# RupertLuo/Valley

Hardware: AMD Instinct MI355X
Metric: frames/sec ViT-L/14 encode + prefill tokens/sec (13B) (higher is better)
Workload: dtype bf16

## Files before the change

valley_amd/csrc/gemm_skinny.hip:

```cpp
#include <cstdlib>
#include "common.hpp"
#include "../../include/valley_hip.h"

namespace {

constexpr int SK_UNROLL = 4;

template <int EPI, int NWV>
__global__ void __launch_bounds__(NWV * 64) gemm_skinny_kernel(const uint16_t* __restrict__ A, const uint16_t* __restrict__ W,
                                                               const float* __restrict__ bias, uint16_t* __restrict__ C, int M, int N,
                                                               int K, int lda, int ldw, int ldc) {
    __shared__ f32x4 red[NWV][4][64];
    const int tid = threadIdx.x, lane = tid & 63, wave = tid >> 6;
    const int l15 = lane & 15, g = lane >> 4;
    const int n0 = blockIdx.x * 32, m0 = blockIdx.y * 32;
    const int kq = K / NWV, kbeg = wave * kq;
    const uint16_t* a0 = A + (size_t)min(m0 + l15, M - 1) * lda + kbeg + g * 8;
    const uint16_t* a1 = A + (size_t)min(m0 + 16 + l15, M - 1) * lda + kbeg + g * 8;
    const uint16_t* w0 = W + (size_t)(n0 + l15) * ldw + kbeg + g * 8;
    const uint16_t* w1 = W + (size_t)(n0 + 16 + l15) * ldw + kbeg + g * 8;
    f32x4 acc[2][2];
#pragma unroll
    for (int i = 0; i < 2; ++i)
#pragma unroll
        for (int j = 0; j < 2; ++j) acc[i][j] = f32x4{0.f, 0.f, 0.f, 0.f};
    const int groups = (kq % (32 * SK_UNROLL) == 0) ? kq / (32 * SK_UNROLL) : 0;
    if (groups > 0) {
        bf16x8 fa0[SK_UNROLL], fa1[SK_UNROLL], fw0[SK_UNROLL], fw1[SK_UNROLL];
        auto load_group = [&](bf16x8 (&xa0)[SK_UNROLL], bf16x8 (&xa1)[SK_UNROLL], bf16x8 (&xw0)[SK_UNROLL], bf16x8 (&xw1)[SK_UNROLL],
                              int k) {
#pragma unroll
            for (int u = 0; u < SK_UNROLL; ++u) {
                xw0[u] = *(const bf16x8*)(w0 + k + 32 * u);
                xw1[u] = *(const bf16x8*)(w1 + k + 32 * u);
                xa0[u] = *(const bf16x8*)(a0 + k + 32 * u);
                xa1[u] = *(const bf16x8*)(a1 + k + 32 * u);
            }
        };
        auto mfma_group = [&](const bf16x8 (&xa0)[SK_UNROLL], const bf16x8 (&xa1)[SK_UNROLL], const bf16x8 (&xw0)[SK_UNROLL],
                              const bf16x8 (&xw1)[SK_UNROLL]) {
#pragma unroll
            for (int u = 0; u < SK_UNROLL; ++u) {
                acc[0][0] = mfma16(xw0[u], xa0[u], acc[0][0]);
                acc[0][1] = mfma16(xw1[u], xa0[u], acc[0][1]);
                acc[1][0] = mfma16(xw0[u], xa1[u], acc[1][0]);
                acc[1][1] = mfma16(xw1[u], xa1[u], acc[1][1]);
            }
        };
        load_group(fa0, fa1, fw0, fw1, 0);
        if constexpr (NWV == 4) {
            bf16x8 ga0[SK_UNROLL], ga1[SK_UNROLL], gw0[SK_UNROLL], gw1[SK_UNROLL];
#pragma unroll 1
            for (int it = 0; it < groups; it += 2) {
                if (it + 1 < groups) load_group(ga0, ga1, gw0, gw1, (it + 1) * 32 * SK_UNROLL);
                mfma_group(fa0, fa1, fw0, fw1);
                if (it + 1 >= groups) break;
                if (it + 2 < groups) load_group(fa0, fa1, fw0, fw1, (it + 2) * 32 * SK_UNROLL);
                mfma_group(ga0, ga1, gw0, gw1);
            }
        } else {
#pragma unroll 1
            for (int it = 0; it < groups; ++it) {
                mfma_group(fa0, fa1, fw0, fw1);
                if (it + 1 < groups) load_group(fa0, fa1, fw0, fw1, (it + 1) * 32 * SK_UNROLL);
            }
        }
    } else
    for (int k = 0; k < kq; k += 32 * SK_UNROLL) {
        bf16x8 fa0[SK_UNROLL], fa1[SK_UNROLL], fw0[SK_UNROLL], fw1[SK_UNROLL];
#pragma unroll
        for (int u = 0; u < SK_UNROLL; ++u) {
            const int kk = min(k + 32 * u, kq - 32);
            fa0[u] = *(const bf16x8*)(a0 + kk);
            fa1[u] = *(const bf16x8*)(a1 + kk);
            fw0[u] = *(const bf16x8*)(w0 + kk);
            fw1[u] = *(const bf16x8*)(w1 + kk);
        }
#pragma unroll
        for (int u = 0; u < SK_UNROLL; ++u) {
            if (k + 32 * u < kq) {
                acc[0][0] = mfma16(fw0[u], fa0[u], acc[0][0]);
                acc[0][1] = mfma16(fw1[u], fa0[u], acc[0][1]);
                acc[1][0] = mfma16(fw0[u], fa1[u], acc[1][0]);
                acc[1][1] = mfma16(fw1[u], fa1[u], acc[1][1]);
            }
        }
    }
#pragma unroll
    for (int i = 0; i < 2; ++i)
#pragma unroll
        for (int j = 0; j < 2; ++j) red[wave][2 * i + j][lane] = acc[i][j];
    __syncthreads();
    if (wave >= 4) return;
    f32x4 v = red[0][wave][lane];
#pragma unroll
    for (int w = 1; w < NWV; ++w) v += red[w][wave][lane];
    const int m = m0 + (wave >> 1) * 16 + l15, n = n0 + (wave & 1) * 16 + 4 * g;
    if (m >= M) return;
    if (bias) v += *(const f32x4*)(bias + n);
    if constexpr (EPI == VLY_EPI_QUICK_GELU) {
#pragma unroll
        for (int r = 0; r < 4; ++r) v[r] = x_sigmoid(v[r], 1.702f);
    }
    if constexpr (EPI == VLY_EPI_RELU) {
#pragma unroll
        for (int r = 0; r < 4; ++r) v[r] = fmaxf(v[r], 0.f);
    }
    u32x2 pk;
    pk[0] = pack_h2(v[0], v[1]);
    pk[1] = pack_h2(v[2], v[3]);
    *(u32x2*)(C + (size_t)m * ldc + n) = pk;
}

}

extern "C" int vly_gemm_skinny_bf16(const void* A, const void* W, const float* bias, void* C, int M, int N, int K, int lda, int ldw,
                                    int ldc, int epilogue, void* stream) {
    if (M <= 0 || M > 256 || N <= 0 || N % 32 || K < 128 || K % 128 || (K >= 2048 && K % 512) || lda % 8 || ldw % 8 || ldc % 4 || ((uintptr_t)A & 15) ||
        ((uintptr_t)W & 15) || ((uintptr_t)C & 7) || (bias && ((uintptr_t)bias & 15))) {
        vly_set_error("vly_gemm_skinny_bf16: unsupported shape/alignment M=%d N=%d K=%d lda=%d ldw=%d ldc=%d", M, N, K, lda, ldw, ldc);
        return -22;
    }
    static const bool narrow_only = getenv("VLY_SKINNY_WAVES") && atoi(getenv("VLY_SKINNY_WAVES")) == 4;
    const bool wide = K >= 2048 && !narrow_only;
    dim3 grid(N / 32, (M + 31) / 32), block(wide ? 1024 : 256);
    hipStream_t st = (hipStream_t)stream;
#define VLY_SKINNY(E)                                                                                                      \
    do {                                                                                                                   \
        if (wide)                                                                                                          \
            hipLaunchKernelGGL((gemm_skinny_kernel<E, 16>), grid, block, 0, st, (const uint16_t*)A, (const uint16_t*)W, bias,  \
                               (uint16_t*)C, M, N, K, lda, ldw, ldc);                                                      \
        else                                                                                                               \
            hipLaunchKernelGGL((gemm_skinny_kernel<E, 4>), grid, block, 0, st, (const uint16_t*)A, (const uint16_t*)W, bias,   \
                               (uint16_t*)C, M, N, K, lda, ldw, ldc);                                                      \
    } while (0)
    switch (epilogue) {
        case VLY_EPI_NONE: VLY_SKINNY(VLY_EPI_NONE); break;
        case VLY_EPI_QUICK_GELU: VLY_SKINNY(VLY_EPI_QUICK_GELU); break;
        case VLY_EPI_RELU: VLY_SKINNY(VLY_EPI_RELU); break;
        default: vly_set_error("vly_gemm_skinny_bf16: unsupported epilogue %d", epilogue); return -22;
    }
#undef VLY_SKINNY
    return vly_check_launch("vly_gemm_skinny_bf16");
}
```

Before: 1717.

## Stage skinny GEMM operands through LDS with direct buffer-to-LDS loads and slot ring

Adds a new skinny GEMM kernel that streams W and A tiles into per-wave LDS rings using buffer_load ... lds with counted vmcnt waits. Operands are then read back through XOR-swizzled LDS addresses. A 16-row M tile variant is used when M is small or the grid is underfilled. This path becomes the default and is meant to replace strided per-lane global vector loads with wide coalesced row loads and deeper prefetch. The trade-off is hand-written inline asm with manual wait counting and a tighter M lower bound (M<=8 now rejected).

```diff
diff --git a/valley_amd/csrc/gemm_skinny.hip b/valley_amd/csrc/gemm_skinny.hip
--- a/valley_amd/csrc/gemm_skinny.hip
+++ b/valley_amd/csrc/gemm_skinny.hip
@@ -112,11 +112,121 @@
     *(u32x2*)(C + (size_t)m * ldc + n) = pk;
 }
 
+template <int EPI, int NWV, int BM, int NSLOT>
+__global__ void __launch_bounds__(NWV * 64) gemm_skinny_lines_kernel(const uint16_t* __restrict__ A, const uint16_t* __restrict__ W,
+                                                                     const float* __restrict__ bias, uint16_t* __restrict__ C, int M, int N,
+                                                                     int K, int lda, int ldw, int ldc) {
+    constexpr int FM = BM / 16;
+    constexpr int PW = 4, PA = BM / 8, PIECES = PW + PA;
+    constexpr int SLOT = PIECES * 1024;
+    static_assert((NSLOT - 1) * PIECES < 64 && NSLOT >= 1 && NSLOT <= 4, "vmcnt is six bits; the counted waits below cover four slots");
+    static_assert(2 * FM * 1024 <= SLOT, "the reduction buffer of a wave lives in its own ring");
+    __shared__ __attribute__((aligned(16))) char ring[NWV][NSLOT][SLOT];
+    const int tid = threadIdx.x, lane = tid & 63, wave = __builtin_amdgcn_readfirstlane(tid >> 6);
+    const int l15 = lane & 15, g = lane >> 4;
+    const int n0 = blockIdx.x * 32, m0 = blockIdx.y * BM;
+    const int kq = K / NWV, kbeg = wave * kq;
+    const int nst = (kq + 63) >> 6;
+    const int r8 = lane >> 3, ch = (lane & 7) ^ r8;
+    const __amdgpu_buffer_rsrc_t rsW = vly_rsrc(W + (size_t)n0 * ldw), rsA = vly_rsrc(A + (size_t)m0 * lda);
+    uint32_t voW[PW], voA[PA];
+#pragma unroll
+    for (int q = 0; q < PW; ++q) voW[q] = ((uint32_t)(q * 8 + r8) * (uint32_t)ldw + (uint32_t)ch * 8u) * 2u;
+#pragma unroll
+    for (int q = 0; q < PA; ++q) voA[q] = ((uint32_t)(min(m0 + q * 8 + r8, M - 1) - m0) * (uint32_t)lda + (uint32_t)ch * 8u) * 2u;
+    const uint32_t half_back = (uint32_t)(ch & 4) * 16u;
+    char* my = &ring[wave][0][0];
+    const uint32_t my_lds = __builtin_amdgcn_readfirstlane((uint32_t)(uintptr_t)(__attribute__((address_space(3))) char*)my);
+    auto dma = [&](uint32_t voff, __amdgpu_buffer_rsrc_t rs, uint32_t soff, uint32_t dst) {
+        asm volatile("s_mov_b32 m0, %3\n\ts_nop 0\n\tbuffer_load_dwordx4 %0, %1, %2 offen lds" ::"v"(voff), "s"(rs), "s"(soff), "s"(dst)
+                     : "memory");
+    };
+    auto issue = [&](int step) {
+        const uint32_t d = my_lds + (uint32_t)(step % NSLOT) * SLOT, soff = (uint32_t)(kbeg + step * 64) * 2u;
+        const uint32_t back = (step * 64 + 32 >= kq) ? half_back : 0u;
+#pragma unroll
+        for (int q = 0; q < PW; ++q) dma(voW[q] - back, rsW, soff, d + q * 1024);
+#pragma unroll
+        for (int q = 0; q < PA; ++q) dma(voA[q] - back, rsA, soff, d + (PW + q) * 1024);
+    };
+    const int rd[2] = {l15 * 128 + (((0 + g) ^ (l15 & 7)) << 4), l15 * 128 + (((4 + g) ^ (l15 & 7)) << 4)};
+    f32x4 acc[FM][2];
+#pragma unroll
+    for (int i = 0; i < FM; ++i)
+#pragma unroll
+        for (int j = 0; j < 2; ++j) acc[i][j] = f32x4{0.f, 0.f, 0.f, 0.f};
+#pragma unroll
+    for (int s = 0; s < NSLOT; ++s)
+        if (s < nst) issue(s);
+#pragma unroll 1
+    for (int i = 0; i < nst; ++i) {
+        const int younger = min(nst - 1 - i, NSLOT - 1);
+        if (NSLOT > 3 && younger == 3) asm volatile("s_waitcnt vmcnt(%0)" ::"i"(NSLOT > 3 ? 3 * PIECES : 0) : "memory");
+        else if (NSLOT > 2 && younger == 2) asm volatile("s_waitcnt vmcnt(%0)" ::"i"(NSLOT > 2 ? 2 * PIECES : 0) : "memory");
+        else if (NSLOT > 1 && younger == 1) asm volatile("s_waitcnt vmcnt(%0)" ::"i"(PIECES) : "memory");
+        else asm volatile("s_waitcnt vmcnt(0)" ::: "memory");
+        const char* s = my + (i % NSLOT) * SLOT;
+        bf16x8 fw[2][2], fa[FM][2];
+#pragma unroll
+        for (int u = 0; u < 2; ++u) {
+#pragma unroll
+            for (int j = 0; j < 2; ++j) fw[j][u] = *(const bf16x8*)(s + j * 2048 + rd[u]);
+#pragma unroll
+            for (int f = 0; f < FM; ++f) fa[f][u] = *(const bf16x8*)(s + PW * 1024 + f * 2048 + rd[u]);
+        }
+        asm volatile("s_waitcnt lgkmcnt(0)" ::: "memory");
+        if (i + NSLOT < nst) issue(i + NSLOT);
+#pragma unroll
+        for (int u = 0; u < 2; ++u) {
+            if (i * 64 + 32 * u < kq) {
+#pragma unroll
+                for (int f = 0; f < FM; ++f)
+#pragma unroll
+                    for (int j = 0; j < 2; ++j) acc[f][j] = mfma16(fw[j][u], fa[f][u], acc[f][j]);
+            }
+        }
+    }
+#pragma unroll
+    for (int f = 0; f < FM; ++f)
+#pragma unroll
+        for (int j = 0; j < 2; ++j) *(f32x4*)(my + (2 * f + j) * 1024 + lane * 16) = acc[f][j];
+    __syncthreads();
+    if (wave >= 2 * FM) return;
+    f32x4 v = *(const f32x4*)(&ring[0][0][0] + wave * 1024 + lane * 16);
+#pragma unroll
+    for (int w = 1; w < NWV; ++w) v += *(const f32x4*)(&ring[w][0][0] + wave * 1024 + lane * 16);
+    const int m = m0 + (wave >> 1) * 16 + l15, n = n0 + (wave & 1) * 16 + 4 * g;
+    if (m >= M) return;
+    if (bias) v += *(const f32x4*)(bias + n);
+    if constexpr (EPI == VLY_EPI_QUICK_GELU) {
+#pragma unroll
+        for (int r = 0; r < 4; ++r) v[r] = x_sigmoid(v[r], 1.702f);
+    }
+    if constexpr (EPI == VLY_EPI_RELU) {
+#pragma unroll
+        for (int r = 0; r < 4; ++r) v[r] = fmaxf(v[r], 0.f);
+    }
+    u32x2 pk;
+    pk[0] = pack_h2(v[0], v[1]);
+    pk[1] = pack_h2(v[2], v[3]);
+    *(u32x2*)(C + (size_t)m * ldc + n) = pk;
+}
+
+#ifndef VLY_SKINNY_SLOTS4_32
+#define VLY_SKINNY_SLOTS4_32 2
+#endif
+#ifndef VLY_SKINNY_SLOTS4_16
+#define VLY_SKINNY_SLOTS4_16 3
+#endif
+#ifndef VLY_SKINNY_BM16
+#define VLY_SKINNY_BM16 1
+#endif
+
 }
 
 extern "C" int vly_gemm_skinny_bf16(const void* A, const void* W, const float* bias, void* C, int M, int N, int K, int lda, int ldw,
                                     int ldc, int epilogue, void* stream) {
-    if (M <= 0 || M > 256 || N <= 0 || N % 32 || K < 128 || K % 128 || (K >= 2048 && K % 512) || lda % 8 || ldw % 8 || ldc % 4 || ((uintptr_t)A & 15) ||
+    if (M <= 8 || M > 256 || N <= 0 || N % 32 || K < 128 || K % 128 || (K >= 2048 && K % 512) || lda % 8 || ldw % 8 || ldc % 4 || ((uintptr_t)A & 15) ||
         ((uintptr_t)W & 15) || ((uintptr_t)C & 7) || (bias && ((uintptr_t)bias & 15))) {
         vly_set_error("vly_gemm_skinny_bf16: unsupported shape/alignment M=%d N=%d K=%d lda=%d ldw=%d ldc=%d", M, N, K, lda, ldw, ldc);
         return -22;
@@ -125,6 +235,34 @@
     const bool wide = K >= 2048 && !narrow_only;
     dim3 grid(N / 32, (M + 31) / 32), block(wide ? 1024 : 256);
     hipStream_t st = (hipStream_t)stream;
+    static const bool lines = [] { const char* e = getenv("VLY_SKINNY_IMPL"); return e ? atoi(e) != 0 : true; }();
+    if (lines && ((size_t)32 * (size_t)(lda > ldw ? lda : ldw) + (size_t)K) * 2 < (1ull << 32)) {
+        const bool bm16 = VLY_SKINNY_BM16 == 1 ? (M <= 16 || (N / 32) * ((M + 31) / 32) < 256) : VLY_SKINNY_BM16 == 2;
+        const dim3 g16(N / 32, (M + 15) / 16);
+#define VLY_SKINNY_L(E)                                                                                                                 \
+    do {                                                                                                                                \
+        if (wide && bm16)                                                                                                               \
+            hipLaunchKernelGGL((gemm_skinny_lines_kernel<E, 16, 16, 1>), g16, block, 0, st, (const uint16_t*)A, (const uint16_t*)W, bias,   \
+                               (uint16_t*)C, M, N, K, lda, ldw, ldc);                                                                   \
+        else if (wide)                                                                                                                  \
+            hipLaunchKernelGGL((gemm_skinny_lines_kernel<E, 16, 32, 1>), grid, block, 0, st, (const uint16_t*)A, (const uint16_t*)W, bias,  \
+                               (uint16_t*)C, M, N, K, lda, ldw, ldc);                                                                   \
+        else if (bm16)                                                                                                                  \
+            hipLaunchKernelGGL((gemm_skinny_lines_kernel<E, 4, 16, VLY_SKINNY_SLOTS4_16>), g16, block, 0, st, (const uint16_t*)A,           \
+                               (const uint16_t*)W, bias, (uint16_t*)C, M, N, K, lda, ldw, ldc);                                         \
+        else                                                                                                                            \
+            hipLaunchKernelGGL((gemm_skinny_lines_kernel<E, 4, 32, VLY_SKINNY_SLOTS4_32>), grid, block, 0, st, (const uint16_t*)A,          \
+                               (const uint16_t*)W, bias, (uint16_t*)C, M, N, K, lda, ldw, ldc);                                         \
+    } while (0)
+        switch (epilogue) {
+            case VLY_EPI_NONE: VLY_SKINNY_L(VLY_EPI_NONE); break;
+            case VLY_EPI_QUICK_GELU: VLY_SKINNY_L(VLY_EPI_QUICK_GELU); break;
+            case VLY_EPI_RELU: VLY_SKINNY_L(VLY_EPI_RELU); break;
+            default: vly_set_error("vly_gemm_skinny_bf16: unsupported epilogue %d", epilogue); return -22;
+        }
+#undef VLY_SKINNY_L
+        return vly_check_launch("vly_gemm_skinny_bf16");
+    }
 #define VLY_SKINNY(E)                                                                                                      \
     do {                                                                                                                   \
         if (wide)                                                                                                          \
```

Result: no change. 1726 (median of 6 runs) (+0.5%).
